# uma-pi1/kge

Measured on AMD Instinct MI355X. Metric: scored triples/sec (1vsAll, ComplEx d=512), higher is better.
Workload: dtype bf16; 1 GPU; FB15k-237 shape ComplEx d=512 1vsAll scoring, bf16 tables, f32 scores: the score_sp and score_po blocks of a batch per step (KgeModel.score_sp_po), batches issued in groups of `group` -- one persistent launch per group (kge_score_queries_multi), which also builds the next group's query vectors; group k on HIP stream k % `group_launches_in_flight`; score rows on a 256-byte pitch; num_entities_per_gpu=14541, num_relations=237, dim=512, batch=512, group=8, group_launches_in_flight=1, parallelism=single GPU, queries=split (q_hi + q_lo)

## Files before the change

kge_amd/csrc/api.hip:

```cpp
#include <dlfcn.h>
#include "common.hpp"
#include "bf16_queries.hpp"
#include <cstdlib>

namespace kge {
int run_tucker3_project(const float* Bm, long long ldb, const Index& idx, const float* W, long long ldw, int d, int dr,
                        long long n, float* out, long long ldo, hipStream_t st);
long long tucker3_bwd_workspace_bytes(int d, int dr, long long n);
int run_tucker3_project_bwd(const float* Bm, long long ldb, const Index& idx, const float* W, long long ldw, int d, int dr,
                            long long n, const float* gout, long long ldg, float* g_brows, long long g_brows_ld,
                            float* g_w, long long g_w_ld, void* ws, long long ws_bytes, hipStream_t st);
int run_rescal_queries(const Operand& A, const Operand* A2, const Operand& R, int dir, int d, long long n, float* q,
                       float* q2, long long q_ld, float* ones, hipStream_t st);
int run_rescal_rows(bool neg_mode, const Operand& S, const Operand& R, const Operand& O, int d, long long n, int slot,
                    const void* neg, int neg_itype, long long neg_ld, long long K, float* out, long long ldo,
                    hipStream_t st);
long long rescal_pairs_bwd_workspace_bytes(int d, long long n);
int run_rescal_pairs_bwd(int dir, const Operand& A, const Operand& R, const Operand& TG, int d, long long n, long long m,
                         const float* gout, long long ldg, float* g_a, float* g_p, float* g_tgt, void* ws,
                         long long ws_bytes, hipStream_t st);
int run_rescal_spo_bwd(const Operand& S, const Operand& R, const Operand& O, int d, long long n, const float* gout,
                       bool accum, float* g_s, long long g_s_ld, float* g_p, long long g_p_ld, float* g_o,
                       long long g_o_ld, hipStream_t st);
int run_rescal_neg_bwd_accum(const Operand& S, const Operand& R, const Operand& O, int d, long long n, int slot,
// ... 339 lines not shown
  return KGE_OK;
}
Operand tgt_op(const kge_tables* t, const kge_index& ix) {
  if (ix.ptr) return ent_op(t, ix);
  const int64_t esize = t->dtype == KGE_BF16 ? 2 : 4;
  return Operand{(const char*)t->ent + (int64_t)ix.start * t->ent_ld * esize, t->ent_ld, Index{nullptr, 1, KGE_I64}};
}
Operand rel_op(const kge_tables* t, const kge_index& ix) {
  return Operand{t->rel, t->rel_ld, make_index(ix)};
}

static bool one_call_prepared(const kge_tables* t, const Operand& TG, int64_t n, int64_t m, int64_t ws_bytes, bool two_sided) {
  const long long e = sw(SW_ONE_CALL_PREPARED);
  if (e == 0) return false;
  if (t->dim != 512 || TG.idx.ptr != nullptr) return false;
  if (ws_bytes < PAIRS_WS_CTRL_BYTES + pairs_bf16_v4_query_bytes((int)t->dim, n, two_sided, false)) return false;
  if (e == 1) return true;
  return two_sided && m >= 2048 && n >= 256;
}

constexpr long long ONE_CALL_V8_ROWS = 512;

static long long one_call_v8_min_rows() {
  const long long v = sw(SW_ONE_CALL_V8_MIN_ROWS);
  if (v >= 2 * ONE_CALL_V8_ROWS) return v;
  return 2 * ONE_CALL_V8_ROWS;
}

static Operand operand_from(const Operand& X, long long k, int esize) {
  Operand r = X;
  if (X.idx.ptr != nullptr)
    r.idx.ptr = (const char*)X.idx.ptr + k * X.idx.stride * (X.idx.itype == KGE_I32 ? 4 : 8);
  else
    r.base = (const char*)X.base + k * X.ld * esize;
  return r;
}

static int one_call_v8(const kge_tables* t, int dir, const Operand& A, const Operand* A2, const Operand& R, const Operand& TG,
                       int64_t n, int64_t m, float* out, int64_t ldo, int64_t b2, void* ws, int64_t ws_bytes, hipStream_t st,
                       int64_t* done) {
  *done = 0;
  if (sw(SW_ONE_CALL_V8) == 0) return KGE_ERR_UNSUPPORTED;
  const bool split = (t->flags & KGE_FLAG_SPLIT_QUERY) != 0, two = A2 != nullptr;
  const int d = (int)t->dim;
  if (t->dtype != KGE_BF16 || (d != 512 && d != 256) || TG.idx.ptr != nullptr || ws == nullptr ||
      n < one_call_v8_min_rows())
    return KGE_ERR_UNSUPPORTED;
  if (d == 256 && m > 65536) return KGE_ERR_UNSUPPORTED;
  if (t->flags & (KGE_FLAG_EXACT | KGE_FLAG_BF16_V3)) return KGE_ERR_UNSUPPORTED;
  if (t->scorer != KGE_COMPLEX && t->scorer != KGE_DISTMULT) return KGE_ERR_UNSUPPORTED;
  if (!pairs_bf16_v4_supported(t->scorer, t->dtype, d, A, R, TG) ||
      (two && !pairs_bf16_v4_supported(t->scorer, t->dtype, d, *A2, R, TG)))
    return KGE_ERR_UNSUPPORTED;
  const long long L = n / ONE_CALL_V8_ROWS;
  const long long per = pairs_bf16_v4_query_bytes(d, ONE_CALL_V8_ROWS, two, split);
  if (L < 2 || L > (1 << 20) || ws_bytes < PAIRS_WS_CTRL_BYTES + L * per || (((uintptr_t)ws + PAIRS_WS_CTRL_BYTES) & 15))
    return KGE_ERR_UNSUPPORTED;
  void* const qf = (char*)ws + PAIRS_WS_CTRL_BYTES;
  int rc = run_query_build_multi(t->scorer, split, A, A2, R, dir, d, ONE_CALL_V8_ROWS, (int)L, qf, per, st);
  if (rc != KGE_OK) return rc;
  rc = run_pairs_bf16_v8(t->scorer, split, TG, two, d, ONE_CALL_V8_ROWS, m, (int)L, qf, per, out, ONE_CALL_V8_ROWS * ldo,
                         ldo, two ? b2 : 0, st, nullptr, NextQ{}, (t->flags >> KGE_FLAG_RESERVE_CUS_SHIFT) & 255);
  if (rc == KGE_OK) *done = L * ONE_CALL_V8_ROWS;
  return rc;
}

static int bf16_store_dispatch(const kge_tables* t, int dir, const Operand& A, const Operand* A2, const Operand& R,
                               const Operand& TG, int64_t n, int64_t m, float* out, int64_t ldo, int64_t b2, void* ws,
                               int64_t ws_bytes, hipStream_t st) {
  if (t->dtype != KGE_BF16 || (t->flags & KGE_FLAG_EXACT)) return KGE_ERR_UNSUPPORTED;
  const int d = (int)t->dim;
  const bool split = (t->flags & KGE_FLAG_SPLIT_QUERY) != 0, two = A2 != nullptr;
  const int reserve = (t->flags >> KGE_FLAG_RESERVE_CUS_SHIFT) & 255;
  {
    int64_t done = 0;
    const int rc8 = one_call_v8(t, dir, A, A2, R, TG, n, m, out, ldo, b2, ws, ws_bytes, st, &done);
    if (rc8 != KGE_ERR_UNSUPPORTED) {
      if (rc8 != KGE_OK || done == n) return rc8;
      const Operand Ar = operand_from(A, done, 2), Rr = operand_from(R, done, 2);
      const Operand A2r = two ? operand_from(*A2, done, 2) : Operand{};
      float* const outr = out + done * ldo;
      const int rcr = bf16_store_dispatch(t, dir, Ar, two ? &A2r : nullptr, Rr, TG, n - done, m, outr, ldo, b2, ws, ws_bytes, st);
      if (rcr != KGE_ERR_UNSUPPORTED || !two) return rcr;
      const int rc = bf16_store_dispatch(t, KGE_SP_, Ar, nullptr, Rr, TG, n - done, m, outr, ldo, 0, ws, ws_bytes, st);
      if (rc) return rc;
      return bf16_store_dispatch(t, KGE_PO_, A2r, nullptr, Rr, TG, n - done, m, outr + b2, ldo, 0, ws, ws_bytes, st);
    }
  }
  const bool v4_ok = ws != nullptr && !(t->flags & KGE_FLAG_BF16_V3) &&
                     pairs_bf16_v4_supported(t->scorer, t->dtype, d, A, R, TG) &&
                     (!two || pairs_bf16_v4_supported(t->scorer, t->dtype, d, *A2, R, TG));
  if (v4_ok && (split || one_call_prepared(t, TG, n, m, ws_bytes, two))) {
    const int rcp = run_pairs_bf16_v4_prepared(t->scorer, split, A, A2, R, TG, dir, d, n, m, out, ldo, two ? b2 : 0, st,
                                               nullptr, nullptr, ws, ws_bytes, reserve, nullptr, nullptr, nullptr, 0, nullptr);
    if (rcp != KGE_ERR_UNSUPPORTED) return rcp;
  }
  if (split) return KGE_ERR_UNSUPPORTED;
  if (v4_ok) {
    const int rc = run_pairs_bf16_v4(t->scorer, A, A2, R, TG, dir, d, n, m, out, ldo, two ? b2 : 0, st, nullptr, ws, ws_bytes,
                                     reserve);
    if (rc != KGE_ERR_UNSUPPORTED) return rc;
  }
  if (!two && pairs_bf16_v3_supported(t->scorer, t->dtype, d, A, R, TG))
    return run_pairs_bf16_v3(t->scorer, A, R, TG, dir, d, n, m, out, ldo, st, nullptr, ws, ws_bytes);
  return KGE_ERR_UNSUPPORTED;
}

int pairs_dispatch(const kge_tables* t, int dir, const Operand& A, const Operand& R,
                   const Operand& TG, int64_t n, int64_t m, float* out, int64_t ldo,
                   void* ws, int64_t ws_bytes, hipStream_t st) {
  const int rc = bf16_store_dispatch(t, dir, A, nullptr, R, TG, n, m, out, ldo, 0, ws, ws_bytes, st);
  if (rc != KGE_ERR_UNSUPPORTED) return rc;
  const bool keep_f32_query = (t->flags & KGE_FLAG_SPLIT_QUERY) && !(t->flags & KGE_FLAG_EXACT) && t->dtype == KGE_BF16;
  return run_pairs_exact(t->scorer, t->dtype, !(t->flags & KGE_FLAG_NO_MFMA), A, R, TG, dir, (int)t->dim, (int)t->rel_dim, n,
                         m, t->l_norm, out, ldo, st, !keep_f32_query);
}

int rescal_contract(const kge_tables* t, int dir, const float* q, const float* ones, const Operand& TG, int64_t n,
                    int64_t m, float* out, int64_t ldo, hipStream_t st) {
  const Index ident{nullptr, 1, KGE_I64};
  const Operand Q{q, t->dim, ident}, ONES{ones, 0, ident};
  return run_pairs_exact(KGE_DISTMULT, KGE_F32, !(t->flags & KGE_FLAG_NO_MFMA), Q, ONES, TG, dir, (int)t->dim, (int)t->dim,
                         n, m, 1.0f, out, ldo, st, true);
}

int pairs_entry(const kge_tables* t, int dir, kge_index a, kge_index p, int64_t n,
                kge_index targets, int64_t m, float* out, int64_t ldo, void* ws, int64_t ws_bytes,
                void* stream) {
  int rc = check_tables(t, true, true, true);
  if (rc) return rc;
  if (n < 0 || m < 0 || (!out && n * m > 0) || ldo < m) return KGE_ERR_INVALID_ARG;
  if (n == 0 || m == 0) return KGE_OK;
  if ((rc = check_index(a, false)) || (rc = check_index(p, false)) || (rc = check_targets(t, targets, m)))
    return rc;
  if (t->scorer == KGE_TRANSH)
    return run_transh_pairs(ent_op(t, a), rel_op(t, p), tgt_op(t, targets), dir, (int)t->dim, n, m, t->l_norm, out, ldo,
                            (hipStream_t)stream);
  if (t->scorer == KGE_RESCAL) {
    if (!ws || ws_bytes < rescal_score_ws_bytes(t, n, 1)) return KGE_ERR_WORKSPACE;
    float* const ones = (float*)ws;
    float* const q = ones + rescal_ones_floats(t);
    rc = run_rescal_queries(ent_op(t, a), nullptr, rel_op(t, p), dir, (int)t->dim, n, q, nullptr, t->dim, ones,
                            (hipStream_t)stream);
    if (rc) return rc;
    return rescal_contract(t, dir, q, ones, tgt_op(t, targets), n, m, out, ldo, (hipStream_t)stream);
  }
  return pairs_dispatch(t, dir, ent_op(t, a), rel_op(t, p), tgt_op(t, targets), n, m, out, ldo,
                        ws, ws_bytes, (hipStream_t)stream);
}

}

namespace kge {
static long long g_switch[SW_COUNT] = {-1, -1, -1, -1, -1, -1, -1, -1, -1, -1, -1, -1, -1, -1, -1, -1, -1, -1, -1, -1};
static_assert(SW_COUNT == 20, "g_switch's initialiser");
static const char* const g_switch_name[SW_COUNT] = {
    "ONE_CALL_PREPARED", "ONE_CALL_V8", "ONE_CALL_V8_MIN_ROWS", "V8_RANK", "RANK_FUSED_FRONT", "BWD_GEMM_LIB",
    "CE_V3", "CE_V8", "V4_OWN_BUILD", "V4_INTERLEAVE", "V4_STORE_SC1", "V6", "V7", "V7_NOSTORE", "V7_PROBE", "V8",
    "V8_VAR", "V8R_PROBE", "TRANSE_GENERIC", "TOPK_COL_TILES"};
long long sw(Switch s) { return __atomic_load_n(&g_switch[(int)s], __ATOMIC_RELAXED); }
static int switch_index(const char* name) {
  if (name == nullptr) return -1;
  if (name[0] == 'K' && name[1] == 'G' && name[2] == 'E' && name[3] == '_') name += 4;
  for (int i = 0; i < SW_COUNT; ++i) {
    const char *a = g_switch_name[i], *b = name;
    while (*a && *a == *b) ++a, ++b;
    if (*a == 0 && *b == 0) return i;
  }
  return -1;
}
}

extern "C" {

int kge_abi_version(void) { return KGE_AMD_ABI_VERSION; }

const char* kge_status_string(int status) {
  switch (status) {
    case KGE_OK: return "ok";
    case KGE_ERR_INVALID_ARG: return "invalid argument";
    case KGE_ERR_UNSUPPORTED: return "unsupported configuration";
    case KGE_ERR_LAUNCH: return "HIP launch/runtime error";
    case KGE_ERR_NO_DEVICE: return "no gfx950 device";
    case KGE_ERR_WORKSPACE: return "workspace too small";
  }
  return "unknown status";
}

int kge_device_count(void) {
  int n = 0;
  if (hipGetDeviceCount(&n) != hipSuccess) {
    (void)hipGetLastError();
    return 0;
  }
  return n;
}

int kge_score_spo(const kge_tables* t, kge_index s, kge_index p, kge_index o, int64_t n,
                  float* out, void* stream) {
  KGE_RANGE();
  int rc = check_tables(t, true, true, true);
  if (rc) return rc;
  if (n < 0 || (!out && n > 0)) return KGE_ERR_INVALID_ARG;
  if (n == 0) return KGE_OK;
  if ((rc = check_index(s, false)) || (rc = check_index(p, false)) ||
      (rc = check_index(o, false)))
    return rc;
  if (t->scorer == KGE_TRANSH)
    return run_transh_spo(false, ent_op(t, s), rel_op(t, p), ent_op(t, o), (int)t->dim, n, 2, nullptr, 0, 0, 0, t->l_norm,
                          out, 0, (hipStream_t)stream);
  if (t->scorer == KGE_RESCAL)
    return run_rescal_rows(false, ent_op(t, s), rel_op(t, p), ent_op(t, o), (int)t->dim, n, 2, nullptr, 0, 0, 0, out, 0,
                           (hipStream_t)stream);
  return run_spo(t->scorer, t->dtype, false, ent_op(t, s), rel_op(t, p), ent_op(t, o),
                 (int)t->dim, (int)t->rel_dim, n, 2, nullptr, 0, 0, 0, t->l_norm, out, 0,
                 (hipStream_t)stream);
}

int64_t kge_score_workspace_bytes(const kge_tables* t, int64_t n) {
  if (t && n > 0 && t->scorer == KGE_RESCAL)
    return check_tables(t, false, false, true) == KGE_OK ? rescal_score_ws_bytes(t, n, 2) : 0;
  if (!t || n <= 0 || t->dtype != KGE_BF16) return 0;
  if (t->scorer != KGE_COMPLEX && t->scorer != KGE_DISTMULT) return 0;
  if (t->dim != 128 && t->dim != 256 && t->dim != 512) return 0;
  if ((t->flags & KGE_FLAG_SPLIT_QUERY) && (t->dim == 256 || t->dim == 512))
    return PAIRS_WS_CTRL_BYTES + pairs_bf16_v4_query_bytes((int)t->dim, n, true, true);
  return pairs_bf16_v3_workspace_bytes((int)t->dim, n);
}

static bool queries_supported(const kge_tables* t) {
  return t->dtype == KGE_BF16 && (t->scorer == KGE_COMPLEX || t->scorer == KGE_DISTMULT) &&
         (t->dim == 256 || t->dim == 512) && !(t->flags & (KGE_FLAG_EXACT |
                                                           KGE_FLAG_BF16_V3));
}

int64_t kge_queries_bytes(const kge_tables* t, int combine, int64_t n) {
  if (!t || n <= 0 || check_tables(t, false) != KGE_OK || !queries_supported(t)) return 0;
  if (combine != KGE_SP_ && combine != KGE_PO_ && combine != KGE_SP_PO) return 0;
  return pairs_bf16_v4_query_bytes((int)t->dim, n, combine == KGE_SP_PO, (t->flags & KGE_FLAG_SPLIT_QUERY) != 0);
}

static int query_operands(const kge_tables* t, int combine, const kge_index& s, const kge_index& p,
                          const kge_index& o, Operand& A, Operand& A2, Operand& R, int& dir) {
  int rc;
  if (combine == KGE_SP_ || combine == KGE_SP_PO) {
    if ((rc = check_index(s, false))) return rc;
  }
  if (combine == KGE_PO_ || combine == KGE_SP_PO) {
    if ((rc = check_index(o, false))) return rc;
  }
  if ((rc = check_index(p, false))) return rc;
  dir = combine == KGE_PO_ ? KGE_PO_ : KGE_SP_;
  A = ent_op(t, combine == KGE_PO_ ? o : s);
  A2 = ent_op(t, o);
  R = rel_op(t, p);
  return KGE_OK;
}

int64_t kge_rescal_queries_bytes(const kge_tables* t, int64_t n) {
  if (!t || n <= 0 || t->scorer != KGE_RESCAL || check_tables(t, false, false, true) != KGE_OK) return 0;
  return n * t->dim * (int64_t)sizeof(float);
}

int kge_rescal_queries(const kge_tables* t, int dir, kge_index a, kge_index p, int64_t n, float* q, int64_t q_ld,
                       void* stream) {
  KGE_RANGE();
  int rc = check_tables(t, true, false, true);
  if (rc) return rc;
  if (t->scorer != KGE_RESCAL) return KGE_ERR_UNSUPPORTED;
  if (dir != KGE_SP_ && dir != KGE_PO_) return KGE_ERR_INVALID_ARG;
  if (n < 0 || (n > 0 && !q) || q_ld < t->dim) return KGE_ERR_INVALID_ARG;
  if (n == 0) return KGE_OK;
  if ((rc = check_index(a, false)) || (rc = check_index(p, false))) return rc;
  return run_rescal_queries(ent_op(t, a), nullptr, rel_op(t, p), dir, (int)t->dim, n, q, nullptr, q_ld, nullptr,
                            (hipStream_t)stream);
}

static int check_tucker3(const kge_tucker3* t, bool need_ptrs) {
  if (!t) return KGE_ERR_INVALID_ARG;
  if (t->dtype != KGE_F32 && t->dtype != KGE_BF16) return KGE_ERR_INVALID_ARG;
  if (t->num_rel <= 0 || t->dim <= 0 || t->base_dim <= 0 || t->dim > (1 << 20)) return KGE_ERR_INVALID_ARG;
  if (t->base_ld < t->base_dim || t->proj_ld < t->base_dim) return KGE_ERR_INVALID_ARG;
  if (need_ptrs && (!t->base || !t->proj)) return KGE_ERR_INVALID_ARG;
  if (t->dtype != KGE_F32 || t->dim > KGE_RESCAL_MAX_DIM || t->base_dim > KGE_TUCKER3_MAX_BASE_DIM)
    return KGE_ERR_UNSUPPORTED;
  return KGE_OK;
}

static int tucker3_index(const kge_tucker3* t, const kge_index& ix, int64_t n, const float** Bm, Index* out) {
  *Bm = (const float*)t->base;
  if (!ix.ptr) {
    if (ix.start < 0 || (int64_t)ix.start + n > t->num_rel) return KGE_ERR_INVALID_ARG;
    *Bm += (int64_t)ix.start * t->base_ld;
    *out = Index{nullptr, 1, KGE_I64};
    return KGE_OK;
  }
  if (ix.start != 0 || (ix.itype != KGE_I32 && ix.itype != KGE_I64) || ix.stride < 1) return KGE_ERR_INVALID_ARG;
  *out = make_index(ix);
  return KGE_OK;
}

int64_t kge_tucker3_project_bytes(const kge_tucker3* t, int64_t n) {
  if (n <= 0 || check_tucker3(t, false) != KGE_OK) return 0;
  return n * t->dim * t->dim * (int64_t)sizeof(float);
}

int kge_tucker3_project(const kge_tucker3* t, kge_index idx, int64_t n, float* out, int64_t out_ld, void* stream) {
  KGE_RANGE();
  int rc = check_tucker3(t, true);
  if (rc) return rc;
  if (n < 0 || (n > 0 && !out) || out_ld < t->dim * t->dim) return KGE_ERR_INVALID_ARG;
  const float* Bm;
// ... 2049 lines not shown
```

kge_amd/csrc/score_pairs_bf16_v8.hip:

```cpp
#include "common.hpp"
#include "bf16_queries.hpp"
#include <atomic>
#include <cstdlib>

namespace kge {

constexpr int V8_UT = 32;
constexpr int V8_BAND_CAP = 255;
constexpr int V8_PB = 14;
constexpr unsigned int V8_DROP = 0x80000000u;

struct V8Args {
  Operand TG;
  long long n, m;
  int rgn1;
  int sides;
  int chunks;
  int nbatch;
  long long q_stride;
  long long out_stride;
  long long out2_off, ldo;
  int nunits, su, wpx;
  float* out;
  const u32x4* qf;
  unsigned long long* dbg;
  NextQ nx;
};

#define KGE_V8_DMA(D, VO, P) \
  KGE_STALL(__LINE__ + 7000); \
  asm volatile("s_mov_b32 m0, %0\n\ts_nop 0\n\tglobal_load_lds_dwordx4 %1, %2" : : "s"(D), "v"(VO), "s"(P) : "memory", "m0")

template <int SCORER, int SPLIT, int AUX, int VAR = 0>
__global__ __launch_bounds__(512, 1) void pairs_bf16_v8_kernel(V8Args a) {
  constexpr int HH = 256;
  constexpr int NKB = 2 * HH / 16;
  constexpr int ROWB = 4 * HH;
  constexpr int UNITB = V8_UT * ROWB;
  constexpr int NBUF = 4;
  constexpr int SMEM = NBUF * UNITB;
  constexpr int RW = SPLIT ? 16 : 32;
  constexpr int NST = SPLIT ? 8 : 16;
  constexpr int PF = SPLIT ? 4 : 8;
  static_assert(NKB % PF == 0 && PF <= 8, "look-ahead depth");
  constexpr int FR0 = 12;
  constexpr int VMN_STEADY = (NST > 15 ? 1 : 0) + NST + 4 + V8_PB / 2;
  constexpr int VMN = VMN_STEADY - 2;
  static_assert(VMN <= (NST > 15 ? 9 : 1) + (NKB - FR0 - 14) + 4 + V8_PB / 2, "the chain behind the cold chain");
  __shared__ __attribute__((aligned(16))) unsigned char smem[SMEM];
  if (a.n < 0) smem[threadIdx.x] = 0;

  const int b = blockIdx.x;
  const int x = b & 7, j = b >> 3;
  const int tid = threadIdx.x, lane = tid & 63;
  const int wave = __builtin_amdgcn_readfirstlane(tid >> 6);
  int u_lo = x * a.su;
  int sux = a.nunits - u_lo;
  if (sux > a.su) sux = a.su;
  const int P = a.nbatch * a.sides * a.chunks;
  const int g0 = 0;
  int g1 = 0, pair0 = 0, pstep = a.wpx;
  if (sux > 0) {
    if (P >= a.wpx) {
      pair0 = j;
      g1 = j < P ? ((P - j + a.wpx - 1) / a.wpx) * sux : 0;
    } else {
      const int nsub = a.wpx / P;
      if (j < P * nsub) {
        pair0 = j % P;
        const int sub = j / P;
        const int lo = (int)((long long)sux * sub / nsub), hi = (int)((long long)sux * (sub + 1) / nsub);
        u_lo += lo;
        sux = hi - lo;
        g1 = sux;
      }
    }
  }

  int dbg_i = 0;
  auto stamp = [&]() {
    if (a.dbg != nullptr && tid == 0 && dbg_i < 32) a.dbg[(long long)blockIdx.x * 64 + dbg_i] = __builtin_readcyclecounter();
    ++dbg_i;
  };
  auto stamp_at = [&](int slot) {
    if (a.dbg != nullptr && tid == 0) a.dbg[(long long)blockIdx.x * 64 + slot] = __builtin_readcyclecounter();
  };

  if (g1 > g0) {
    stamp();
    const unsigned char* const tgb = (const unsigned char*)a.TG.base;
    const long long tld2 = a.TG.ld * 2;
    const long long m = a.m;
    const unsigned int lane16 = (unsigned int)lane << 4;
    const int r4 = 4 * wave;
    const unsigned int dx0 = (unsigned int)((r4 & 15) << 4);
    int dq = g0;
    int du = g0 % sux;
    const int ulast = (g1 - 1) % sux;
    auto dma_piece = [&](int un, int ks, auto kc) __attribute__((always_inline)) {
      constexpr int kk = decltype(kc)::value;
      long long r = (long long)(u_lo + un) * V8_UT + r4 + kk;
      if (r >= m) r = m - 1;
      const unsigned char* pk = tgb + r * tld2;
      const unsigned int dk = (unsigned int)((ks & (NBUF - 1)) * UNITB + (r4 + kk) * ROWB);
      const unsigned int vo = lane16 ^ (dx0 + (unsigned int)(kk << 4));
      KGE_V8_DMA(dk, vo, pk);
    };
    auto dma_advance = [&]() __attribute__((always_inline)) {
      ++dq;
      if (++du == sux) du = 0;
    };
    auto fill_unit = [&](int k) __attribute__((always_inline)) {
      const int un = dq < g1 ? du : ulast;
      v4_static_for<0, 4>([&](auto kc) __attribute__((always_inline)) { dma_piece(un, k, kc); });
      dma_advance();
    };

    const int fi = lane & 31, fh = lane >> 5;
    bf16x8 afr[NKB];
    unsigned int bp[8];
#pragma unroll
    for (int t = 0; t < 8; ++t) bp[t] = (unsigned int)(fi * ROWB + (((2 * t + fh) ^ (fi & 15)) << 4));
    bf16x8 bq[PF];
    auto bread = [&](bf16x8& dst, auto kc) __attribute__((always_inline)) {
      constexpr int kb = decltype(kc)::value;
      const unsigned int addr = bp[kb & 7];
      asm volatile("ds_read_b128 %0, %1 offset:%2" : "=v"(dst) : "v"(addr), "i"((kb >> 3) * 256) : "memory");
    };
    const unsigned int ldo4 = (unsigned int)(a.ldo * 4);
    const unsigned int svo = (unsigned int)(((long long)(4 * fh) * a.ldo + fi) * 4);
    __amdgpu_buffer_rsrc_t srs = __builtin_amdgcn_make_buffer_rsrc((void*)a.out, 0, 0, 0x00020000);
    auto store_q = [&](const f32x16& acc, auto qc, unsigned int vo, unsigned int colb) __attribute__((always_inline)) {
      constexpr int q = decltype(qc)::value;
      constexpr int r = SPLIT ? (q & 3) + 8 * (q >> 2) : q;
      constexpr int rowc = SPLIT ? 8 * (r >> 3) + (r & 3) : 8 * (r >> 2) + (r & 3);
      const unsigned int vr = vo + (unsigned int)rowc * ldo4;
      float v = acc[r];
      if constexpr (SPLIT) {
        const float lo = acc[r + 4];
        v = v + lo;
      }
      if constexpr (VAR & 1) {
        asm volatile("" : : "v"(v), "v"(vr));
      } else {
        __builtin_amdgcn_raw_buffer_store_b32(__builtin_bit_cast(unsigned int, v), srs, vr, colb, AUX);
      }
    };
    auto unit_vo = [&](int cu, unsigned int& colb) __attribute__((always_inline)) -> unsigned int {
      const long long col0 = (long long)(u_lo + cu) * V8_UT;
      colb = (unsigned int)(col0 * 4);
      return (col0 + V8_UT <= m || col0 + fi < m) ? svo : V8_DROP;
    };

    f32x16 acc0, acc1;
    auto chain = [&](int ks, f32x16& acc, const f32x16& prev, unsigned int vo, unsigned int colb, auto cold, auto&& frag)
        __attribute__((always_inline)) {
      constexpr bool COLD = decltype(cold)::value;
      const unsigned int bdelta = ((ks + 1) & (NBUF - 1)) ? (unsigned int)UNITB : (unsigned int)(-(NBUF - 1) * UNITB);
      int un = dq < g1 ? du : ulast;
      v4_static_for<0, NKB>([&](auto kc) __attribute__((always_inline)) {
        constexpr int kb = decltype(kc)::value;
        asm volatile("s_waitcnt lgkmcnt(%0)" ::"i"(PF - 1) : "memory");
        if constexpr (kb == V8_PB) {
          asm volatile("s_waitcnt vmcnt(%0)" ::"i"(COLD ? 25 : VMN) : "memory");
          KGE_BARRIER();
        }
        __builtin_amdgcn_sched_barrier(0);
        if constexpr (kb == 0) {
          const f32x16 zero = {0, 0, 0, 0, 0, 0, 0, 0, 0, 0, 0, 0, 0, 0, 0, 0};
          acc = __builtin_amdgcn_mfma_f32_32x32x16_bf16(afr[0], bq[0], zero, 0, 0, 0);
        } else {
          acc = __builtin_amdgcn_mfma_f32_32x32x16_bf16(afr[kb], bq[kb % PF], acc, 0, 0, 0);
        }
        if constexpr (kb + PF == NKB) {
#pragma unroll
          for (int t = 0; t < 8; ++t) asm volatile("v_add_u32 %0, %1, %0" : "+v"(bp[t]) : "s"(bdelta));
        }
        bread(bq[kb % PF], std::integral_constant<int, (kb + PF) % NKB>{});
        if constexpr ((kb & 1) == 0 && kb / 2 < NST) store_q(prev, std::integral_constant<int, kb / 2>{}, vo, colb);
        if constexpr (COLD && kb < NKB - FR0) frag(std::integral_constant<int, FR0 + kb>{});
        if constexpr (COLD && kb < 14 && (kb & 3) == 1) dma_piece(un, ks + 2, std::integral_constant<int, kb / 4>{});
        if constexpr (COLD && kb == 14) {
          dma_advance();
          un = dq < g1 ? du : ulast;
        }
        if constexpr (kb >= 17 && ((kb - 17) & 3) == 0) dma_piece(un, ks + 3, std::integral_constant<int, (kb - 17) / 4>{});
      });
      dma_advance();
      stamp();
    };
    using Cold = std::true_type;
    using Warm = std::false_type;
    auto nofrag = [](auto) {};

    int g = g0, ks = 0;
    int pair = pair0;
    const int cu = 0;
    bool first = true;
    while (g < g1) {
      const int cnt = sux;
      const int per = a.sides * a.chunks;
      const int lb = pair / per, rem = pair - lb * per;
      const int side = rem / a.chunks, ch = rem - side * a.chunks;
      const long long rb = (long long)ch * (8 * RW) + RW * wave;
      long long rows_here = rb < a.n ? (a.n - rb < RW ? a.n - rb : RW) : 0;
      float* const ob = a.out + (long long)lb * a.out_stride + (side ? a.out2_off : 0) + (rows_here > 0 ? rb : 0) * a.ldo;
      srs = __builtin_amdgcn_make_buffer_rsrc((void*)ob, 0, (int)(rows_here * a.ldo * 4), 0x00020000);
      int grp = 2 * ch + (wave >> 2);
      if (grp >= a.rgn1) grp = a.rgn1 - 1;
      grp += side * a.rgn1;
      const unsigned char* const gbase = (const unsigned char*)(a.qf + (long long)lb * a.q_stride + (long long)grp * 4 * NKB * 64);
      unsigned int flo;
      const unsigned char* fb;
      int frange;
      if constexpr (SPLIT) {
        const int part = (fi >> 3) & 1, rr = 16 * (wave & 3) + 8 * (fi >> 4) + (fi & 7);
        flo = (unsigned int)((((2 * part + (rr >> 5)) * NKB) * 64 + (rr & 31) + 32 * fh) * 16);
        fb = gbase;
        frange = 4 * NKB * 1024;
      } else {
        flo = (unsigned int)(lane * 16);
        fb = gbase + (wave & 3) * (NKB * 1024);
        frange = NKB * 1024;
      }
      const __amdgpu_buffer_rsrc_t frs = __builtin_amdgcn_make_buffer_rsrc((void*)fb, 0, frange, 0x00020000);
      auto load_fragments = [&](auto lo, auto hi) __attribute__((always_inline)) {
        v4_static_for<decltype(lo)::value, decltype(hi)::value>([&](auto kc) __attribute__((always_inline)) {
          constexpr int kb = decltype(kc)::value;
          afr[kb] = __builtin_bit_cast(bf16x8, __builtin_amdgcn_raw_buffer_load_b128(frs, flo + kb * 1024, 0, 16 ));
        });
      };
      using C0 = std::integral_constant<int, 0>;
      using CF = std::integral_constant<int, FR0>;
      using C32 = std::integral_constant<int, NKB>;
      unsigned int pvo = V8_DROP, pcolb = 0;
      if (first) {
        fill_unit(0);
        load_fragments(C0{}, CF{});
        asm volatile("s_waitcnt vmcnt(%0)" ::"i"(FR0) : "memory");
        KGE_BARRIER();
        stamp();
        fill_unit(1);
        v4_static_for<0, PF>([&](auto jc) __attribute__((always_inline)) { bread(bq[decltype(jc)::value], jc); });
        first = false;
        chain(ks, acc0, acc1, pvo, pcolb, Cold{}, [&](auto kc) __attribute__((always_inline)) {
          load_fragments(kc, std::integral_constant<int, decltype(kc)::value + 1>{});
        });
      } else {
        load_fragments(C0{}, C32{});
        chain(ks, acc0, acc1, pvo, pcolb, Warm{}, nofrag);
      }
      pvo = unit_vo(cu, pcolb);
      ++ks;
      int i = 1;
      for (; i + 1 < cnt; i += 2) {
        chain(ks, acc1, acc0, pvo, pcolb, Warm{}, nofrag);
        pvo = unit_vo(cu + i, pcolb);
        chain(ks + 1, acc0, acc1, pvo, pcolb, Warm{}, nofrag);
        pvo = unit_vo(cu + i + 1, pcolb);
        ks += 2;
      }
      if (i < cnt) {
        chain(ks, acc1, acc0, pvo, pcolb, Warm{}, nofrag);
        pvo = unit_vo(cu + i, pcolb);
        ++ks;
        v4_static_for<0, NST>([&](auto qc) __attribute__((always_inline)) { store_q(acc1, qc, pvo, pcolb); });
      } else {
        v4_static_for<0, NST>([&](auto qc) __attribute__((always_inline)) { store_q(acc0, qc, pvo, pcolb); });
      }
      g += cnt;
      pair += pstep;
    }
    asm volatile("s_waitcnt lgkmcnt(0)" ::: "memory");
    if constexpr (PF == 8)
      asm volatile("" : : "v"(bq[0]), "v"(bq[1]), "v"(bq[2]), "v"(bq[3]), "v"(bq[4]), "v"(bq[5]), "v"(bq[6]), "v"(bq[7]));
    else
      asm volatile("" : : "v"(bq[0]), "v"(bq[1]), "v"(bq[2]), "v"(bq[3]));
    stamp_at(34);
  }
  if (a.nx.qf != nullptr)
    v4_build_queries<SCORER, HH, SPLIT>(a.nx, (long long)blockIdx.x * 512 + threadIdx.x, (long long)gridDim.x * 512);
}

void v6_set_stamps(unsigned long long* p);
unsigned long long* v6_get_stamps();

int run_pairs_bf16_v8_store256(const Operand& TG, bool split, bool two_sided, long long n, long long m, int nbatch,
                               const void* qf, long long q_stride_bytes, float* out, long long out_stride, long long ldo,
                               long long out2_off, int sc1, int reserve_cus, hipStream_t st);

static int v8_cu_count() {
  static std::atomic<int> cache[64];
  int dev = 0;
  if (hipGetDevice(&dev) != hipSuccess) return 0;
  if (dev >= 0 && dev < 64) {
    const int c = cache[dev].load(std::memory_order_relaxed);
    if (c > 0) return c;
  }
  int v = 0;
  if (hipDeviceGetAttribute(&v, hipDeviceAttributeMultiprocessorCount, dev) != hipSuccess) return 0;
  if (dev >= 0 && dev < 64) cache[dev].store(v, std::memory_order_relaxed);
  return v;
}

static int g_v8_launches[2] = {0, 0};
int v8_launch_count(int which) { return (which == 0 || which == 1) ? __atomic_load_n(&g_v8_launches[which], __ATOMIC_RELAXED) : -1; }

template <int SCORER, int SPLIT>
static int launch_v8(V8Args& a, int sc1, hipStream_t st) {
  int cus = v8_cu_count();
  (void)cus;
  __atomic_fetch_add(&g_v8_launches[0], 1, __ATOMIC_RELAXED);
  const dim3 grid(8 * a.wpx), block(512);
#ifdef KGE_V8_PROBES
  if constexpr (SCORER == KGE_COMPLEX && SPLIT == 1) {
    if (sw(SW_V8_VAR) == 1) {
      hipLaunchKernelGGL((pairs_bf16_v8_kernel<SCORER, SPLIT, 2, 1>), grid, block, 0, st, a);
      return hipGetLastError() == hipSuccess ? KGE_OK : KGE_ERR_LAUNCH;
    }
  }
#endif
  if (sc1 == 1)
    hipLaunchKernelGGL((pairs_bf16_v8_kernel<SCORER, SPLIT, 16>), grid, block, 0, st, a);
  else if (sc1 == 2)
    hipLaunchKernelGGL((pairs_bf16_v8_kernel<SCORER, SPLIT, 2>), grid, block, 0, st, a);
  else if (sc1 == 3)
    hipLaunchKernelGGL((pairs_bf16_v8_kernel<SCORER, SPLIT, 18>), grid, block, 0, st, a);
  else
    hipLaunchKernelGGL((pairs_bf16_v8_kernel<SCORER, SPLIT, 0>), grid, block, 0, st, a);
  return hipGetLastError() == hipSuccess ? KGE_OK : KGE_ERR_LAUNCH;
}

int run_pairs_bf16_v8(int scorer, bool split, const Operand& TG, bool two_sided, int d, long long n, long long m,
                      int nbatch, const void* qf, long long q_stride_bytes, float* out, long long out_stride,
                      long long ldo, long long out2_off, hipStream_t st, unsigned long long* dbg, const NextQ& nx,
                      int reserve_cus) {
  if ((d != 512 && d != 256) || TG.idx.ptr != nullptr || qf == nullptr || nbatch < 1) return KGE_ERR_UNSUPPORTED;
  const long long e = sw(SW_V8);
  if (e == 0) return KGE_ERR_UNSUPPORTED;
  if (nbatch == 1 && e != 1) return KGE_ERR_UNSUPPORTED;
  if (TG.ld * 2 >= (1LL << 28) || ldo >= (1LL << 24)) return KGE_ERR_UNSUPPORTED;
  if ((q_stride_bytes & 15) || ((uintptr_t)qf & 15)) return KGE_ERR_INVALID_ARG;
  const long long rgr = split ? 64 : 128;
  const long long rgn1 = (n + rgr - 1) / rgr;
  const long long pairs = (long long)nbatch * (two_sided ? 2 : 1) * ((rgn1 + 1) / 2);
  const long long nunits = (m + V8_UT - 1) / V8_UT;
  if (rgn1 > (1 << 20) || pairs * nunits >= (1LL << 30)) return KGE_ERR_UNSUPPORTED;
  int cus = v8_cu_count() - reserve_cus;
  if (cus > 256) cus = 256;
  if (cus < 8) cus = 8;
  V8Args a{};
  a.TG = TG;
  a.n = n;
  a.m = m;
  a.rgn1 = (int)rgn1;
  a.sides = two_sided ? 2 : 1;
  a.chunks = (int)((rgn1 + 1) / 2);
  a.nbatch = nbatch;
  a.q_stride = q_stride_bytes / 16;
  a.out_stride = out_stride;
  a.out2_off = out2_off;
  a.ldo = ldo;
  a.nunits = (int)nunits;
  a.su = (int)((nunits + 7) / 8);
  a.wpx = cus / 8;
  a.out = out;
  a.qf = (const u32x4*)qf;
  a.dbg = dbg != nullptr ? dbg : v6_get_stamps();
  a.nx = nx;
  const long long sc1e = sw(SW_V4_STORE_SC1);
  const bool st_aligned = (ldo & 7) == 0 && (out2_off & 7) == 0 && (out_stride & 7) == 0 && ((uintptr_t)out & 31) == 0;
  const double bytes = (double)nbatch * (double)n * (double)m * 4.0 * (two_sided ? 2 : 1);
  const int sc1 = sc1e >= 0 ? (int)sc1e : (!st_aligned ? 0 : (bytes > 160e6 ? 2 : (bytes <= 48e6 ? 1 : 0)));
  if (d == 256) {
    if (nx.qf != nullptr) return KGE_ERR_INVALID_ARG;
    const int pol = sc1e >= 0 ? (int)(sc1e & 3) : (st_aligned && bytes > 1e9 ? 1 : 0);
    const int rc = run_pairs_bf16_v8_store256(TG, split, two_sided, n, m, nbatch, qf, q_stride_bytes, out, out_stride, ldo,
                                              out2_off, pol, reserve_cus, st);
    if (rc == KGE_OK) __atomic_fetch_add(&g_v8_launches[0], 1, __ATOMIC_RELAXED);
    return rc;
  }
#define KGE_V8L(SC) return split ? launch_v8<SC, 1>(a, sc1, st) : launch_v8<SC, 0>(a, sc1, st)
  if (scorer == KGE_COMPLEX) { KGE_V8L(KGE_COMPLEX); }
  if (scorer == KGE_DISTMULT) { KGE_V8L(KGE_DISTMULT); }
#undef KGE_V8L
  return KGE_ERR_UNSUPPORTED;
}


struct V8RankArgs {
  Operand TG;
  long long n, m;
  int rgn1, sides, chunks;
  int nunits, su, wpx;
  const u32x4* qf;
  unsigned long long* dbg;
  CeArgs ce;
};

template <int SCORER, int HH, int SPLIT, int PROBE = 0, int BAND = 0>
__global__ __launch_bounds__(512, 1) void pairs_bf16_v8_rank_kernel(V8RankArgs a) {
  static_assert(!BAND || !SPLIT, "the band launch runs the q_hi chains only");
  constexpr bool DUP = SPLIT && HH == 256;
  constexpr int PARTS = (SPLIT && HH == 128) ? 2 : 1;
  constexpr int FSETS = PARTS;
  constexpr int NT = (HH == 128 && !SPLIT) ? 2 : 1;
  constexpr int NACC = NT * PARTS;
  constexpr int UT = V8_UT * NT;
  constexpr int NKB = 2 * HH / 16;
  constexpr int ROWB = 4 * HH;
  constexpr int SPR = ROWB / 16;
  constexpr int RPP = 64 / SPR;
  constexpr int UNITB = UT * ROWB;
  constexpr int SUBB = V8_UT * ROWB;
  constexpr int NBUF = 4;
  constexpr int SMEM = NBUF * UNITB;
  constexpr int NP = UNITB / 1024 / 8;
  constexpr int RW = DUP ? 16 : 32;
  constexpr int PF = 4;
  constexpr int PB = NKB == 32 ? 14 : 6;
  constexpr bool RAWFAST = HH == 128;
  __shared__ __attribute__((aligned(16))) unsigned char smem[SMEM];
  if (a.n < 0) smem[threadIdx.x] = 0;

  const int b = blockIdx.x;
  const int x = b & 7, j = b >> 3;
  const int tid = threadIdx.x, lane = tid & 63;
  const int wave = __builtin_amdgcn_readfirstlane(tid >> 6);
  int u_lo = x * a.su;
  int sux = a.nunits - u_lo;
  if (sux > a.su) sux = a.su;
  const int P = a.sides * a.chunks;
  const int g0 = 0;
  int g1 = 0, pair0 = 0, pstep = a.wpx;
  if (sux > 0) {
    if (P >= a.wpx) {
      pair0 = j;
      g1 = j < P ? ((P - j + a.wpx - 1) / a.wpx) * sux : 0;
    } else {
      const int nsub = a.wpx / P;
      if (j < P * nsub) {
        pair0 = j % P;
        const int sub = j / P;
        const int lo = (int)((long long)sux * sub / nsub), hi = (int)((long long)sux * (sub + 1) / nsub);
        u_lo += lo;
        sux = hi - lo;
        g1 = sux;
      }
    }
  }
  if (g1 <= g0) return;
  int dbg_i = 0;
  auto stamp = [&]() {
    if (a.dbg != nullptr && tid == 0 && dbg_i < 32) a.dbg[(long long)blockIdx.x * 64 + dbg_i] = __builtin_readcyclecounter();
    ++dbg_i;
  };
  stamp();
  if (a.dbg != nullptr && tid == 0) a.dbg[(long long)blockIdx.x * 64 + 42] = wall_clock64();

  const unsigned char* const tgb = (const unsigned char*)a.TG.base;
  const long long tld2 = a.TG.ld * 2;
  const long long m = a.m;
  const int lr = lane / SPR, slot = lane % SPR;
  const int rp0 = wave * NP * RPP;
  int dq = g0, du = g0 % sux;
  const int ulast = (g1 - 1) % sux;
  auto dma_piece = [&](int un, int ks, auto kc) __attribute__((always_inline)) {
    constexpr int kk = decltype(kc)::value;
    const int ru = rp0 + kk * RPP;
    const long long r0 = (long long)(u_lo + un) * UT + ru;
    const unsigned int dk = (unsigned int)((ks & (NBUF - 1)) * UNITB + ru * ROWB);
    const unsigned int sw = (unsigned int)((slot ^ ((ru + lr) & 15)) << 4);
    const long long rb = r0 < m ? r0 : m - 1;
    const unsigned char* pk = tgb + rb * tld2;
    unsigned int vo = sw;
    if constexpr (RPP > 1) {
      const int left = (int)(m - 1 - rb < RPP - 1 ? m - 1 - rb : RPP - 1);
      vo += (unsigned int)((lr < left ? lr : left) * (int)tld2);
    }
    KGE_V8_DMA(dk, vo, pk);
  };
  auto dma_advance = [&]() __attribute__((always_inline)) {
// ... 747 lines not shown
```

kge_amd/csrc/switches.hpp:

```cpp
#pragma once

namespace kge {

enum Switch : int {
  SW_ONE_CALL_PREPARED = 0,
  SW_ONE_CALL_V8,
  SW_ONE_CALL_V8_MIN_ROWS,
  SW_V8_RANK,
  SW_RANK_FUSED_FRONT,
  SW_BWD_GEMM_LIB,
  SW_CE_V3,
  SW_CE_V8,
  SW_V4_OWN_BUILD,
  SW_V4_INTERLEAVE,
  SW_V4_STORE_SC1,
  SW_V6,
  SW_V7,
  SW_V7_NOSTORE,
  SW_V7_PROBE,
  SW_V8,
  SW_V8_VAR,
  SW_V8R_PROBE,
  SW_TRANSE_GENERIC,
  SW_TOPK_COL_TILES,
  SW_COUNT
};

long long sw(Switch s);

}
```

Measured before the change: 552.9 billion scored triples/s.

## Use 16x16x32 MFMA chains with paired b64 stores for split-query v8 scoring

For split (hi+lo) queries, the v8 pairs kernel now uses 16x16x32 bf16 MFMA tiles, two accumulators per hi/lo part, in place of 32x32x16 tiles. Fragment layout, LDS read offsets, counted vmcnt waits and the output mapping are all reworked to match. Each lane now writes two adjacent columns with one 64-bit buffer store, and a scalar fallback handles an odd tail column. The aim is fewer store instructions and a shorter MFMA dependency latency, at the cost of more MFMA issues and a more complex edge path. A switch restores the old 32x32 path, and probe timestamps are added under a compile flag.

```diff
diff --git a/kge_amd/csrc/api.hip b/kge_amd/csrc/api.hip
--- a/kge_amd/csrc/api.hip
+++ b/kge_amd/csrc/api.hip
@@ -515,12 +515,12 @@
 }
 
 namespace kge {
-static long long g_switch[SW_COUNT] = {-1, -1, -1, -1, -1, -1, -1, -1, -1, -1, -1, -1, -1, -1, -1, -1, -1, -1, -1, -1};
-static_assert(SW_COUNT == 20, "g_switch's initialiser");
+static long long g_switch[SW_COUNT] = {-1, -1, -1, -1, -1, -1, -1, -1, -1, -1, -1, -1, -1, -1, -1, -1, -1, -1, -1, -1, -1};
+static_assert(SW_COUNT == 21, "g_switch's initialiser");
 static const char* const g_switch_name[SW_COUNT] = {
     "ONE_CALL_PREPARED", "ONE_CALL_V8", "ONE_CALL_V8_MIN_ROWS", "V8_RANK", "RANK_FUSED_FRONT", "BWD_GEMM_LIB",
     "CE_V3", "CE_V8", "V4_OWN_BUILD", "V4_INTERLEAVE", "V4_STORE_SC1", "V6", "V7", "V7_NOSTORE", "V7_PROBE", "V8",
-    "V8_VAR", "V8R_PROBE", "TRANSE_GENERIC", "TOPK_COL_TILES"};
+    "V8_VAR", "V8_MFMA32", "V8R_PROBE", "TRANSE_GENERIC", "TOPK_COL_TILES"};
 long long sw(Switch s) { return __atomic_load_n(&g_switch[(int)s], __ATOMIC_RELAXED); }
 static int switch_index(const char* name) {
   if (name == nullptr) return -1;
diff --git a/kge_amd/csrc/score_pairs_bf16_v8.hip b/kge_amd/csrc/score_pairs_bf16_v8.hip
--- a/kge_amd/csrc/score_pairs_bf16_v8.hip
+++ b/kge_amd/csrc/score_pairs_bf16_v8.hip
@@ -31,8 +31,14 @@
   KGE_STALL(__LINE__ + 7000); \
   asm volatile("s_mov_b32 m0, %0\n\ts_nop 0\n\tglobal_load_lds_dwordx4 %1, %2" : : "s"(D), "v"(VO), "s"(P) : "memory", "m0")
 
-template <int SCORER, int SPLIT, int AUX, int VAR = 0>
+struct V8Acc16 {
+  f32x4 a[2][2];
+};
+
+template <int SCORER, int SPLIT, int AUX, int VAR = 0, int MS = 0>
 __global__ __launch_bounds__(512, 1) void pairs_bf16_v8_kernel(V8Args a) {
+  static_assert(MS == 0 || (MS == 1 && SPLIT), "16x16x32 chains: split queries only");
+  constexpr bool M16 = MS != 0;
   constexpr int HH = 256;
   constexpr int NKB = 2 * HH / 16;
   constexpr int ROWB = 4 * HH;
@@ -40,13 +46,17 @@
   constexpr int NBUF = 4;
   constexpr int SMEM = NBUF * UNITB;
   constexpr int RW = SPLIT ? 16 : 32;
-  constexpr int NST = SPLIT ? 8 : 16;
+  constexpr int NST = M16 ? 4 : SPLIT ? 8 : 16;
   constexpr int PF = SPLIT ? 4 : 8;
   static_assert(NKB % PF == 0 && PF <= 8, "look-ahead depth");
   constexpr int FR0 = 12;
-  constexpr int VMN_STEADY = (NST > 15 ? 1 : 0) + NST + 4 + V8_PB / 2;
-  constexpr int VMN = VMN_STEADY - 2;
-  static_assert(VMN <= (NST > 15 ? 9 : 1) + (NKB - FR0 - 14) + 4 + V8_PB / 2, "the chain behind the cold chain");
+  constexpr int NST_LO = NST < V8_PB / 2 ? NST : V8_PB / 2;
+  constexpr int VMN_STEADY = (NST > 15 ? 1 : 0) + NST + 4 + NST_LO;
+  constexpr int VMN = M16 ? VMN_STEADY : VMN_STEADY - 2;
+  static_assert(VMN == (M16 ? 12 : SPLIT ? 17 : 26), "counted wait of the unit barrier");
+  static_assert(VMN <= (NST - NST_LO) + (NKB - FR0 - 14) + 4 + NST_LO, "the chain behind the cold chain");
+  constexpr int VMN_COLD = NST_LO + V8_PB + 4;
+  static_assert(VMN_COLD == (M16 ? 22 : 25), "counted wait of the cold chain");
   __shared__ __attribute__((aligned(16))) unsigned char smem[SMEM];
   if (a.n < 0) smem[threadIdx.x] = 0;
 
@@ -88,6 +98,12 @@
 
   if (g1 > g0) {
     stamp();
+#ifdef KGE_V8_PROBES
+    if (a.dbg != nullptr && tid == 0) {
+      a.dbg[(long long)blockIdx.x * 64 + 48] = __builtin_readcyclecounter();
+      a.dbg[(long long)blockIdx.x * 64 + 49] = wall_clock64();
+    }
+#endif
     const unsigned char* const tgb = (const unsigned char*)a.TG.base;
     const long long tld2 = a.TG.ld * 2;
     const long long m = a.m;
@@ -119,8 +135,16 @@
     const int fi = lane & 31, fh = lane >> 5;
     bf16x8 afr[NKB];
     unsigned int bp[8];
-#pragma unroll
-    for (int t = 0; t < 8; ++t) bp[t] = (unsigned int)(fi * ROWB + (((2 * t + fh) ^ (fi & 15)) << 4));
+    const int mt = lane & 15, mg = lane >> 4;
+#pragma unroll
+    for (int t = 0; t < 8; ++t) {
+      if constexpr (M16) {
+        const int row = 2 * mt + (t & 1);
+        bp[t] = (unsigned int)(row * ROWB + (((4 * (t >> 1) + mg) ^ (row & 15)) << 4));
+      } else {
+        bp[t] = (unsigned int)(fi * ROWB + (((2 * t + fh) ^ (fi & 15)) << 4));
+      }
+    }
     bf16x8 bq[PF];
     auto bread = [&](bf16x8& dst, auto kc) __attribute__((always_inline)) {
       constexpr int kb = decltype(kc)::value;
@@ -128,32 +152,63 @@
       asm volatile("ds_read_b128 %0, %1 offset:%2" : "=v"(dst) : "v"(addr), "i"((kb >> 3) * 256) : "memory");
     };
     const unsigned int ldo4 = (unsigned int)(a.ldo * 4);
-    const unsigned int svo = (unsigned int)(((long long)(4 * fh) * a.ldo + fi) * 4);
+    using Acc = std::conditional_t<M16, V8Acc16, f32x16>;
+    const unsigned int svo =
+        M16 ? (unsigned int)(((long long)(4 * mg) * a.ldo + 2 * mt) * 4) : (unsigned int)(((long long)(4 * fh) * a.ldo + fi) * 4);
     __amdgpu_buffer_rsrc_t srs = __builtin_amdgcn_make_buffer_rsrc((void*)a.out, 0, 0, 0x00020000);
-    auto store_q = [&](const f32x16& acc, auto qc, unsigned int vo, unsigned int colb) __attribute__((always_inline)) {
+    auto store_q = [&](const Acc& acc, auto qc, unsigned int vo, unsigned int colb) __attribute__((always_inline)) {
       constexpr int q = decltype(qc)::value;
-      constexpr int r = SPLIT ? (q & 3) + 8 * (q >> 2) : q;
-      constexpr int rowc = SPLIT ? 8 * (r >> 3) + (r & 3) : 8 * (r >> 2) + (r & 3);
-      const unsigned int vr = vo + (unsigned int)rowc * ldo4;
-      float v = acc[r];
-      if constexpr (SPLIT) {
-        const float lo = acc[r + 4];
-        v = v + lo;
-      }
-      if constexpr (VAR & 1) {
-        asm volatile("" : : "v"(v), "v"(vr));
+      if constexpr (M16) {
+        const unsigned int vr = vo + (unsigned int)q * ldo4;
+        const float h0 = acc.a[0][0][q], l0 = acc.a[1][0][q], h1 = acc.a[0][1][q], l1 = acc.a[1][1][q];
+        float v0 = h0 + l0, v1 = h1 + l1;
+        asm("" : "+v"(v0));
+        if constexpr (VAR & 1) {
+          asm volatile("" : : "v"(v0), "v"(v1), "v"(vr));
+        } else {
+          const u32x2 v = {__builtin_bit_cast(unsigned int, v0), __builtin_bit_cast(unsigned int, v1)};
+          __builtin_amdgcn_raw_buffer_store_b64(v, srs, vr, colb, AUX);
+        }
       } else {
-        __builtin_amdgcn_raw_buffer_store_b32(__builtin_bit_cast(unsigned int, v), srs, vr, colb, AUX);
+        constexpr int r = SPLIT ? (q & 3) + 8 * (q >> 2) : q;
+        constexpr int rowc = SPLIT ? 8 * (r >> 3) + (r & 3) : 8 * (r >> 2) + (r & 3);
+        const unsigned int vr = vo + (unsigned int)rowc * ldo4;
+        float v = acc[r];
+        if constexpr (SPLIT) {
+          const float lo = acc[r + 4];
+          v = v + lo;
+        }
+        if constexpr (VAR & 1) {
+          asm volatile("" : : "v"(v), "v"(vr));
+        } else {
+          __builtin_amdgcn_raw_buffer_store_b32(__builtin_bit_cast(unsigned int, v), srs, vr, colb, AUX);
+        }
       }
     };
     auto unit_vo = [&](int cu, unsigned int& colb) __attribute__((always_inline)) -> unsigned int {
       const long long col0 = (long long)(u_lo + cu) * V8_UT;
       colb = (unsigned int)(col0 * 4);
+      if constexpr (M16) return (col0 + V8_UT <= m || col0 + 2 * mt + 1 < m) ? svo : V8_DROP;
       return (col0 + V8_UT <= m || col0 + fi < m) ? svo : V8_DROP;
     };
-
-    f32x16 acc0, acc1;
-    auto chain = [&](int ks, f32x16& acc, const f32x16& prev, unsigned int vo, unsigned int colb, auto cold, auto&& frag)
+    auto flush_unit = [&](const Acc& acc, int cuu, unsigned int vo, unsigned int colb) __attribute__((always_inline)) {
+      v4_static_for<0, NST>([&](auto qc) __attribute__((always_inline)) { store_q(acc, qc, vo, colb); });
+      if constexpr (M16 && !(VAR & 1)) {
+        const long long col0 = (long long)(u_lo + cuu) * V8_UT;
+        if (col0 + V8_UT > m && (m & 1)) {
+          const unsigned int lvo = (col0 + 2 * mt + 1 == m) ? svo : V8_DROP;
+#pragma unroll
+          for (int q = 0; q < 4; ++q) {
+            const float h0 = acc.a[0][0][q], l0 = acc.a[1][0][q];
+            const float v0 = h0 + l0;
+            __builtin_amdgcn_raw_buffer_store_b32(__builtin_bit_cast(unsigned int, v0), srs, lvo + (unsigned int)q * ldo4, colb, AUX);
+          }
+        }
+      }
+    };
+
+    Acc acc0, acc1;
+    auto chain = [&](int ks, Acc& acc, const Acc& prev, unsigned int vo, unsigned int colb, auto cold, auto&& frag)
         __attribute__((always_inline)) {
       constexpr bool COLD = decltype(cold)::value;
       const unsigned int bdelta = ((ks + 1) & (NBUF - 1)) ? (unsigned int)UNITB : (unsigned int)(-(NBUF - 1) * UNITB);
@@ -162,11 +217,21 @@
         constexpr int kb = decltype(kc)::value;
         asm volatile("s_waitcnt lgkmcnt(%0)" ::"i"(PF - 1) : "memory");
         if constexpr (kb == V8_PB) {
-          asm volatile("s_waitcnt vmcnt(%0)" ::"i"(COLD ? 25 : VMN) : "memory");
+          asm volatile("s_waitcnt vmcnt(%0)" ::"i"(COLD ? VMN_COLD : VMN) : "memory");
           KGE_BARRIER();
         }
         __builtin_amdgcn_sched_barrier(0);
-        if constexpr (kb == 0) {
+        if constexpr (M16) {
+          constexpr int sj = kb >> 1, sc = kb & 1;
+          if constexpr (sj == 0) {
+            const f32x4 zero = {0, 0, 0, 0};
+            acc.a[0][sc] = __builtin_amdgcn_mfma_f32_16x16x32_bf16(afr[0], bq[kb % PF], zero, 0, 0, 0);
+            acc.a[1][sc] = __builtin_amdgcn_mfma_f32_16x16x32_bf16(afr[1], bq[kb % PF], zero, 0, 0, 0);
+          } else {
+            acc.a[0][sc] = __builtin_amdgcn_mfma_f32_16x16x32_bf16(afr[2 * sj], bq[kb % PF], acc.a[0][sc], 0, 0, 0);
+            acc.a[1][sc] = __builtin_amdgcn_mfma_f32_16x16x32_bf16(afr[2 * sj + 1], bq[kb % PF], acc.a[1][sc], 0, 0, 0);
+          }
+        } else if constexpr (kb == 0) {
           const f32x16 zero = {0, 0, 0, 0, 0, 0, 0, 0, 0, 0, 0, 0, 0, 0, 0, 0};
           acc = __builtin_amdgcn_mfma_f32_32x32x16_bf16(afr[0], bq[0], zero, 0, 0, 0);
         } else {
@@ -213,7 +278,12 @@
       unsigned int flo;
       const unsigned char* fb;
       int frange;
-      if constexpr (SPLIT) {
+      if constexpr (M16) {
+        const int rr = 16 * (wave & 3) + mt;
+        flo = (unsigned int)(((((rr >> 5) * NKB) + (mg >> 1)) * 64 + (rr & 31) + 32 * (mg & 1)) * 16);
+        fb = gbase;
+        frange = 4 * NKB * 1024;
+      } else if constexpr (SPLIT) {
         const int part = (fi >> 3) & 1, rr = 16 * (wave & 3) + 8 * (fi >> 4) + (fi & 7);
         flo = (unsigned int)((((2 * part + (rr >> 5)) * NKB) * 64 + (rr & 31) + 32 * fh) * 16);
         fb = gbase;
@@ -227,7 +297,8 @@
       auto load_fragments = [&](auto lo, auto hi) __attribute__((always_inline)) {
         v4_static_for<decltype(lo)::value, decltype(hi)::value>([&](auto kc) __attribute__((always_inline)) {
           constexpr int kb = decltype(kc)::value;
-          afr[kb] = __builtin_bit_cast(bf16x8, __builtin_amdgcn_raw_buffer_load_b128(frs, flo + kb * 1024, 0, 16 ));
+          constexpr int fo = M16 ? (kb & 1) * (2 * NKB * 1024) + (kb >> 1) * 2048 : kb * 1024;
+          afr[kb] = __builtin_bit_cast(bf16x8, __builtin_amdgcn_raw_buffer_load_b128(frs, flo + fo, 0, 16 ));
         });
       };
       using C0 = std::integral_constant<int, 0>;
@@ -264,9 +335,9 @@
         chain(ks, acc1, acc0, pvo, pcolb, Warm{}, nofrag);
         pvo = unit_vo(cu + i, pcolb);
         ++ks;
-        v4_static_for<0, NST>([&](auto qc) __attribute__((always_inline)) { store_q(acc1, qc, pvo, pcolb); });
+        flush_unit(acc1, cu + i, pvo, pcolb);
       } else {
-        v4_static_for<0, NST>([&](auto qc) __attribute__((always_inline)) { store_q(acc0, qc, pvo, pcolb); });
+        flush_unit(acc0, cu + cnt - 1, pvo, pcolb);
       }
       g += cnt;
       pair += pstep;
@@ -277,6 +348,12 @@
     else
       asm volatile("" : : "v"(bq[0]), "v"(bq[1]), "v"(bq[2]), "v"(bq[3]));
     stamp_at(34);
+#ifdef KGE_V8_PROBES
+    if (a.dbg != nullptr && tid == 0) {
+      a.dbg[(long long)blockIdx.x * 64 + 50] = __builtin_readcyclecounter();
+      a.dbg[(long long)blockIdx.x * 64 + 51] = wall_clock64();
+    }
+#endif
   }
   if (a.nx.qf != nullptr)
     v4_build_queries<SCORER, HH, SPLIT>(a.nx, (long long)blockIdx.x * 512 + threadIdx.x, (long long)gridDim.x * 512);
@@ -315,19 +392,34 @@
 #ifdef KGE_V8_PROBES
   if constexpr (SCORER == KGE_COMPLEX && SPLIT == 1) {
     if (sw(SW_V8_VAR) == 1) {
-      hipLaunchKernelGGL((pairs_bf16_v8_kernel<SCORER, SPLIT, 2, 1>), grid, block, 0, st, a);
+      if (sw(SW_V8_MFMA32) == 1)
+        hipLaunchKernelGGL((pairs_bf16_v8_kernel<SCORER, SPLIT, 2, 1>), grid, block, 0, st, a);
+      else
+        hipLaunchKernelGGL((pairs_bf16_v8_kernel<SCORER, SPLIT, 2, 1, 1>), grid, block, 0, st, a);
       return hipGetLastError() == hipSuccess ? KGE_OK : KGE_ERR_LAUNCH;
     }
   }
 #endif
+  const int ms = SPLIT && sw(SW_V8_MFMA32) != 1 ? 1 : 0;
+#define KGE_V8_GO(AUXV)                                                                               \
+  do {                                                                                                \
+    if constexpr (SPLIT) {                                                                            \
+      if (ms == 1) {                                                                                  \
+        hipLaunchKernelGGL((pairs_bf16_v8_kernel<SCORER, SPLIT, AUXV, 0, 1>), grid, block, 0, st, a); \
+        break;                                                                                        \
+      }                                                                                               \
+    }                                                                                                 \
+    hipLaunchKernelGGL((pairs_bf16_v8_kernel<SCORER, SPLIT, AUXV>), grid, block, 0, st, a);           \
+  } while (0)
   if (sc1 == 1)
-    hipLaunchKernelGGL((pairs_bf16_v8_kernel<SCORER, SPLIT, 16>), grid, block, 0, st, a);
+    KGE_V8_GO(16);
   else if (sc1 == 2)
-    hipLaunchKernelGGL((pairs_bf16_v8_kernel<SCORER, SPLIT, 2>), grid, block, 0, st, a);
+    KGE_V8_GO(2);
   else if (sc1 == 3)
-    hipLaunchKernelGGL((pairs_bf16_v8_kernel<SCORER, SPLIT, 18>), grid, block, 0, st, a);
+    KGE_V8_GO(18);
   else
-    hipLaunchKernelGGL((pairs_bf16_v8_kernel<SCORER, SPLIT, 0>), grid, block, 0, st, a);
+    KGE_V8_GO(0);
+#undef KGE_V8_GO
   return hipGetLastError() == hipSuccess ? KGE_OK : KGE_ERR_LAUNCH;
 }
 
diff --git a/kge_amd/csrc/switches.hpp b/kge_amd/csrc/switches.hpp
--- a/kge_amd/csrc/switches.hpp
+++ b/kge_amd/csrc/switches.hpp
@@ -20,6 +20,7 @@
   SW_V7_PROBE,
   SW_V8,
   SW_V8_VAR,
+  SW_V8_MFMA32,
   SW_V8R_PROBE,
   SW_TRANSE_GENERIC,
   SW_TOPK_COL_TILES,
```

Measured after the change: 597.1 billion scored triples/s, median of 6. +8.0%, better.
